# spaceandtimefdn/blitzar

Hardware: NVIDIA H100
Metric: MSM throughput (scalar*point terms/sec), ristretto255, n=2^20 per GPU (higher is better)
Workload: dtype u32 limbs (integer modular arithmetic)

## Files before the change

### blitzar_b200/csrc/msm.cuh

```cuda
#pragma once
#include <algorithm>
#include <vector>

#include "batch_affine.cuh"
#include "curve.cuh"
#include "engine_api.cuh"
#include "lanefield.cuh"

namespace b200 {

struct ColumnDesc {
  const unsigned char* base;
  u64 row_stride;
  u32 bit_offset;
  u32 bit_width;
  u32 n;
  u32 is_signed;
  u32 first_window;
  u32 num_windows;
  u32 table_n;
  u32 gen_base;
};
B200_HD u32 bucket_windows(const ColumnDesc& col) { return col.table_n ? (col.num_windows ? 1u : 0u) : col.num_windows; }

B200_HD void load_scalar_bits(u32 v[8], bool& negative, const ColumnDesc& col, u64 i) {
  const unsigned char* row = col.base + i * col.row_stride;
#pragma unroll
  for (int k = 0; k < 8; ++k)
    v[k] = 0;
  const u32 width = col.bit_width;
  const unsigned char* p = row + (col.bit_offset >> 3);
  const u32 sh = col.bit_offset & 7u;
  if (sh == 0 && width == 256 && (((size_t)p) & 15u) == 0) {
    const uint4* q = (const uint4*)p;
    uint4 a = q[0], b = q[1];
    v[0] = a.x; v[1] = a.y; v[2] = a.z; v[3] = a.w;
    v[4] = b.x; v[5] = b.y; v[6] = b.z; v[7] = b.w;
  } else if (sh == 0 && (width & 31u) == 0 && (((size_t)p) & 3u) == 0) {
    const u32* q = (const u32*)p;
#pragma unroll
    for (int k = 0; k < 8; ++k)
      if ((u32)k < (width >> 5))
        v[k] = q[k];
  } else {
    const u32 nbytes = (sh + width + 7u) >> 3;
#pragma unroll
    for (int k = 0; k < 8; ++k) {
      u64 acc = 0;
#pragma unroll
      for (int b = 0; b < 5; ++b) {
        u32 idx = 4u * k + b;
        if (idx < nbytes)
          acc |= (u64)p[idx] << (8 * b);
      }
      v[k] = (u32)(acc >> sh);
    }
#pragma unroll
    for (int k = 0; k < 8; ++k) {
      int lo = 32 * k;
      if ((int)width <= lo)
        v[k] = 0;
      else if ((int)width < lo + 32)
        v[k] &= (1u << (width - lo)) - 1u;
    }
  }
  negative = false;
  if (col.is_signed) {
    u32 top = width - 1;
    bool neg = false;
#pragma unroll
    for (int k = 0; k < 8; ++k)
      if ((top >> 5) == (u32)k)
        neg = (v[k] >> (top & 31u)) & 1u;
    if (neg) {
      u64 c = 1;
#pragma unroll
      for (int k = 0; k < 8; ++k) {
        int lo = 32 * k;
        u32 m = 0;
        if ((int)width >= lo + 32)
          m = 0xffffffffu;
        else if ((int)width > lo)
          m = (1u << (width - lo)) - 1u;
        c += (u64)((~v[k]) & m);
        v[k] = (u32)c & m;
        c = (m == 0xffffffffu) ? (c >> 32) : 0;
      }
      negative = true;
    }
  }
}

constexpr u32 kAllWindows = 0xffffffffu;
template <class Fn>
B200_HD void for_each_digit(const u32 v[8], bool negative, const ColumnDesc& col, u32 c,
                            u32 nbuckets, Fn f, u32 only_window = kAllWindows) {
  const u32 half = nbuckets;
  const u32 mask = (1u << c) - 1u;
  u64 buf = 0;
  u32 nb = 0, w = 0, carry = 0;
  const u32 W = only_window == kAllWindows
                    ? col.num_windows
                    : (only_window < col.num_windows ? only_window + 1 : 0u);
#pragma unroll
  for (int k = 0; k < 8; ++k) {
    buf |= (u64)v[k] << nb;
    nb += 32;
    while (nb >= c && w < W) {
      u32 d = ((u32)buf & mask) + carry;
      buf >>= c;
      nb -= c;
      bool dneg = d > half;
      carry = dneg ? 1u : 0u;
      if (dneg)
        d = (1u << c) - d;
      if (d && (only_window == kAllWindows || w == only_window))
        f((col.first_window + (col.table_n ? 0u : w)) * nbuckets + (d - 1u), negative != dneg, w);
      ++w;
    }
  }
  while (w < W) {
    u32 d = ((u32)buf & mask) + carry;
    buf >>= c;
    bool dneg = d > half;
    carry = dneg ? 1u : 0u;
    if (dneg)
      d = (1u << c) - d;
    if (d && (only_window == kAllWindows || w == only_window))
      f((col.first_window + (col.table_n ? 0u : w)) * nbuckets + (d - 1u), negative != dneg, w);
    ++w;
  }
}

B200_HD u32 column_of(const u64* col_start, u32 ncols, u64 tid) {
  u32 lo = 0, hi = ncols;
  while (hi - lo > 1) {
    const u32 mid = (lo + hi) >> 1;
    if (tid >= col_start[mid])
      lo = mid;
    else
      hi = mid;
  }
  return lo;
}
struct CountBody {
  static constexpr int kBlock = 256;
  const ColumnDesc* cols;
  const u64* col_start;
  u32 ncols, c, nbuckets;
  u32* counts;
  B200_HD void operator()(u64 tid) const {
    const u32 j = column_of(col_start, ncols, tid);
    const ColumnDesc col = cols[j];
    u64 i = tid - col_start[j];
    u32 v[8];
    bool neg;
    load_scalar_bits(v, neg, col, i);
    u32* cnt = counts;
    for_each_digit(v, neg, col, c, nbuckets, [cnt](u32 key, bool, u32) { B200_ATOMIC_ADD(&cnt[key], 1u); });
  }
};

struct ScatterBody {
  static constexpr int kBlock = 256;
  const ColumnDesc* cols;
  const u64* col_start;
  u32 ncols, c, nbuckets;
  u32* cursor;
  u64* entries;
  u64 total_terms;
  B200_HD void operator()(u64 tid) const {
    u32 only = kAllWindows;
    if (total_terms) {
      only = (u32)(tid / total_terms);
      tid -= (u64)only * total_terms;
    }
    const u32 j = column_of(col_start, ncols, tid);
    const ColumnDesc col = cols[j];
    if (only != kAllWindows && only >= col.num_windows)
      return;
    u64 i = tid - col_start[j];
    u32 v[8];
    bool neg;
    load_scalar_bits(v, neg, col, i);
    u32* cur = cursor;
    u64* en = entries;
    const u32 ii = (u32)i + col.gen_base, tn = col.table_n;
    for_each_digit(v, neg, col, c, nbuckets, [cur, en, ii, tn](u32 key, bool negate, u32 w) {
      u32 pos = B200_ATOMIC_ADD(&cur[key], 1u);
      en[pos] = ((u64)key << 32) | (u64)(((ii + w * tn) << 1) | (negate ? 1u : 0u));
    }, only);
  }
};

constexpr u32 kScanChunk = 256, kScanChunkFirst = 64;
struct ScanUpBody {
  static constexpr int kBlock = 128;
  const u32* in;
  u64 n;
  u32* partial;
  u32 chunk;
  B200_HD void operator()(u64 t) const {
    u64 b = t * chunk, e = b + chunk < n ? b + chunk : n;
    u32 s = 0;
    for (u64 i = b; i < e; ++i)
      s += in[i];
    partial[t] = s;
  }
};
struct ScanTopBody {
  static constexpr int kBlock = 32;
  u32* data;
  u64 n;
  B200_HD void operator()(u64) const {
    u32 s = 0;
    for (u64 i = 0; i < n; ++i) {
      u32 v = data[i];
      data[i] = s;
      s += v;
    }
  }
};
struct ScanDownBody {
  static constexpr int kBlock = 128;
  u32* data;
  u64 n;
  const u32* partial_scanned;
  u32 chunk;
  B200_HD void operator()(u64 t) const {
    u64 b = t * chunk, e = b + chunk < n ? b + chunk : n;
    u32 s = partial_scanned[t];
    for (u64 i = b; i < e; ++i) {
      u32 v = data[i];
      data[i] = s;
      s += v;
    }
  }
};

inline void exclusive_scan(u32* data, u64 n, stream_t s, u32 chunk = kScanChunkFirst) {
  if (n <= kScanChunk) {
    launch(ScanTopBody{data, n}, 1, s);
    return;
  }
  u64 m = (n + chunk - 1) / chunk;
  u32* partial = (u32*)dev_alloc(m * sizeof(u32), s);
  launch(ScanUpBody{data, n, partial, chunk}, m, s);
  exclusive_scan(partial, m, s, kScanChunk);
  launch(ScanDownBody{data, n, partial, chunk}, m, s);
  dev_free(partial, s);
}

#if defined(__CUDACC__) && !defined(B200_EMULATE)
#define B200_BINNED_SORT 1
constexpr u32 kMicroBins = 16384, kBinCap = 8192, kBinSpan = 4096, kMaxBinShift = 12;
constexpr u64 kBinnedSortMinEntries = 1ull << 20;

template <int kBlock> __device__ u32 block_exclusive_scan(u32 v, u32* warp_sums, u32* total) {
  const u32 lane = threadIdx.x & 31u, warp = threadIdx.x >> 5;
  u32 x = v;
#pragma unroll
  for (int d = 1; d < 32; d <<= 1) {
    const u32 y = __shfl_up_sync(0xffffffffu, x, d);
    if (lane >= (u32)d)
      x += y;
  }
  if (lane == 31)
    warp_sums[warp] = x;
  __syncthreads();
  if (warp == 0) {
    u32 w = lane < kBlock / 32 ? warp_sums[lane] : 0u;
#pragma unroll
    for (int d = 1; d < 32; d <<= 1) {
      const u32 y = __shfl_up_sync(0xffffffffu, w, d);
      if (lane >= (u32)d)
        w += y;
    }
    if (lane < kBlock / 32)
      warp_sums[lane] = w;
  }
  __syncthreads();
  const u32 pre = (warp ? warp_sums[warp - 1] : 0u) + x - v;
  *total = warp_sums[kBlock / 32 - 1];
  __syncthreads();
  return pre;
}

template <class Fn>
__device__ void for_each_entry(const ColumnDesc* cols, const u64* col_start, u32 ncols, u32 c,
                               u32 nbuckets, u64 tid, Fn f) {
  const u32 j = column_of(col_start, ncols, tid);
  const ColumnDesc col = cols[j];
  const u64 i = tid - col_start[j];
  u32 v[8];
  bool neg;
  load_scalar_bits(v, neg, col, i);
  const u32 ii = (u32)i + col.gen_base, tn = col.table_n;
  for_each_digit(v, neg, col, c, nbuckets, [&](u32 key, bool negate, u32 w) {
    f(key, ((u64)key << 32) | (u64)(((ii + w * tn) << 1) | (negate ? 1u : 0u)));
  });
}

struct MicroCountBody {
  static constexpr int kBlock = 512;
  const ColumnDesc* cols;
  const u64* col_start;
  u32 ncols, c, nbuckets;
  u64 total_terms;
  u32 tile, shift, nmicro;
  u32* micro_counts;
  __device__ void run(u32 b, unsigned char* smem) const {
    u32* h = (u32*)smem;
    for (u32 m = threadIdx.x; m < nmicro; m += kBlock)
      h[m] = 0;
    __syncthreads();
    const u64 lo = (u64)b * tile, hi = lo + tile < total_terms ? lo + tile : total_terms;
    const u32 sh = shift;
    for (u64 t = lo + threadIdx.x; t < hi; t += kBlock)
      for_each_entry(cols, col_start, ncols, c, nbuckets, t,
                     [h, sh](u32 key, u64) { atomicAdd(&h[key >> sh], 1u); });
    __syncthreads();
    for (u32 m = threadIdx.x; m < nmicro; m += kBlock)
      if (h[m])
        atomicAdd(&micro_counts[m], h[m]);
  }
};

struct PlanBinsBody {
  static constexpr int kBlock = 1024;
  const u32* micro_counts;
  u32 nmicro, span_micro;
  u64 nkeys;
  u32* bin_of;
  u32* bin_start;
  u32* bin_micro;
  u32* bin_cursor;
  u32* nbins_out;
  u32* counts;
  u32* d_m;
  __device__ bool starts_bin(const u32* st, u32 m) const {
    constexpr u32 H = kBinCap / 2;
    return m == 0 || m % span_micro == 0 || micro_counts[m] > H || micro_counts[m - 1] > H ||
           st[m] / H != st[m - 1] / H;
  }
  __device__ void run(u32, unsigned char* smem) const {
    __shared__ u32 ws[32];
    u32* st = (u32*)smem;
    const u32 per = (nmicro + kBlock - 1) / kBlock, m0 = min(threadIdx.x * per, nmicro),
              m1 = min(m0 + per, nmicro);
    u32 sum = 0;
    for (u32 m = m0; m < m1; ++m)
      sum += micro_counts[m];
    u32 total;
    u32 run = block_exclusive_scan<kBlock>(sum, ws, &total);
    for (u32 m = m0; m < m1; ++m) {
      st[m] = run;
      run += micro_counts[m];
    }
    __syncthreads();
    u32 nf = 0;
    for (u32 m = m0; m < m1; ++m)
      nf += starts_bin(st, m) ? 1u : 0u;
    u32 nbins;
    u32 id = block_exclusive_scan<kBlock>(nf, ws, &nbins);
    for (u32 m = m0; m < m1; ++m) {
      if (starts_bin(st, m)) {
        bin_start[id] = st[m];
        bin_micro[id] = m;
        bin_cursor[id] = st[m];
        ++id;
      }
      bin_of[m] = id - 1;
    }
    if (threadIdx.x == 0) {
      bin_start[nbins] = total;
      bin_micro[nbins] = nmicro;
      *nbins_out = nbins;
      counts[nkeys] = total;
      d_m[0] = total;
    }
  }
};

struct CoarseScatterBody {
  static constexpr int kBlock = 1024;
  const ColumnDesc* cols;
  const u64* col_start;
  u32 ncols, c, nbuckets;
  u64 total_terms;
  u32 tile, shift, nmicro;
  const u32* bin_of;
  const u32* nbins_ptr;
  u32* bin_cursor;
  u64* tmp;
  __device__ void run(u32 b, unsigned char* smem) const {
    __shared__ u32 ws[32];
    u32* h = (u32*)smem;
    u32* delta = h + nmicro;
    u64* stage = (u64*)(delta + nmicro + (nmicro & 1u));
    const u32 nbins = *nbins_ptr;
    for (u32 k = threadIdx.x; k < nbins; k += kBlock)
      h[k] = 0;
    __syncthreads();
    const u64 lo = (u64)b * tile, hi = lo + tile < total_terms ? lo + tile : total_terms;
    const u32 sh = shift;
    const u32* map = bin_of;
    for (u64 t = lo + threadIdx.x; t < hi; t += kBlock)
      for_each_entry(cols, col_start, ncols, c, nbuckets, t,
                     [h, sh, map](u32 key, u64) { atomicAdd(&h[__ldg(&map[key >> sh])], 1u); });
    __syncthreads();
    const u32 per = (nbins + kBlock - 1) / kBlock, k0 = min(threadIdx.x * per, nbins),
              k1 = min(k0 + per, nbins);
    u32 sum = 0;
    for (u32 k = k0; k < k1; ++k)
      sum += h[k];
    u32 size;
    u32 run = block_exclusive_scan<kBlock>(sum, ws, &size);
    for (u32 k = k0; k < k1; ++k) {
      const u32 n = h[k];
      if (n)
        delta[k] = atomicAdd(&bin_cursor[k], n) - run;
      h[k] = run;
      run += n;
    }
    __syncthreads();
    for (u64 t = lo + threadIdx.x; t < hi; t += kBlock)
      for_each_entry(cols, col_start, ncols, c, nbuckets, t, [h, sh, map, stage](u32 key, u64 e) {
        stage[atomicAdd(&h[__ldg(&map[key >> sh])], 1u)] = e;
      });
    __syncthreads();
    for (u32 i = threadIdx.x; i < size; i += kBlock) {
      const u64 e = stage[i];
      tmp[delta[__ldg(&map[(u32)(e >> 32) >> sh])] + i] = e;
    }
  }
};

struct BinSortBody {
  static constexpr int kBlock = 1024;
  static constexpr size_t kSmem = 2 * kBinCap * sizeof(u64) + kBinSpan * sizeof(u32);
  const u64* tmp;
  const u32* bin_start;
  const u32* bin_micro;
  const u32* nbins_ptr;
  u32 shift;
  u64 nkeys;
  u64* entries;
  u32* counts;
  __device__ void run(u32 b, unsigned char* smem) const {
    __shared__ u32 ws[32];
    if (b >= *nbins_ptr)
      return;
    u64* ent = (u64*)smem;
    u32* h = (u32*)(smem + 2 * kBinCap * sizeof(u64));
    const u32 lo = bin_start[b], size = bin_start[b + 1] - lo;
    const u64 klo = (u64)bin_micro[b] << shift, khi_m = (u64)bin_micro[b + 1] << shift;
    const u32 span = (u32)((khi_m < nkeys ? khi_m : nkeys) - klo);
    const bool local = size <= kBinCap;
    for (u32 k = threadIdx.x; k < span; k += kBlock)
      h[k] = 0;
    if (local) {
#pragma unroll 4
      for (u32 i = threadIdx.x; i < size; i += kBlock)
        ent[i] = tmp[(u64)lo + i];
    }
    __syncthreads();
    for (u32 i = threadIdx.x; i < size; i += kBlock) {
      const u64 e = local ? ent[i] : tmp[(u64)lo + i];
      atomicAdd(&h[(u32)(e >> 32) - (u32)klo], 1u);
    }
    __syncthreads();
    const u32 per = (span + kBlock - 1) / kBlock, k0 = min(threadIdx.x * per, span),
              k1 = min(k0 + per, span);
    u32 sum = 0;
    for (u32 k = k0; k < k1; ++k)
      sum += h[k];
    u32 total;
    u32 run = block_exclusive_scan<kBlock>(sum, ws, &total);
    for (u32 k = k0; k < k1; ++k) {
      const u32 n = h[k];
      h[k] = run;
      run += n;
      counts[klo + k] = lo + run;
    }
    __syncthreads();
    if (!local) {
      for (u32 i = threadIdx.x; i < size; i += kBlock) {
        const u64 e = tmp[(u64)lo + i];
        entries[(u64)lo + atomicAdd(&h[(u32)(e >> 32) - (u32)klo], 1u)] = e;
      }
      return;
    }
    u64* sorted = ent + kBinCap;
    for (u32 i = threadIdx.x; i < size; i += kBlock) {
      const u64 e = ent[i];
      sorted[atomicAdd(&h[(u32)(e >> 32) - (u32)klo], 1u)] = e;
    }
    __syncthreads();
    for (u32 i = threadIdx.x; i < size; i += kBlock)
      entries[(u64)lo + i] = sorted[i];
  }
};

inline u32 binned_sort_shift(u64 nkeys) {
  u32 shift = 0;
  while ((nkeys + (1ull << shift) - 1) >> shift > kMicroBins)
    ++shift;
  return shift;
}

inline void binned_sort(stream_t s, const ColumnDesc* d_cols, const u64* d_col_start, u32 ncols,
                        u32 c, u32 nbuckets, u64 total_terms, u64 max_entries, u32 max_windows,
                        u64 nkeys, u64* entries, u32* counts, u32* d_m) {
  const u32 shift = binned_sort_shift(nkeys);
  const u32 nmicro = (u32)((nkeys + (1ull << shift) - 1) >> shift);
  const u32 span_micro = std::max(1u, kBinSpan >> shift);
  u32* ws = (u32*)dev_alloc((5ull * nmicro + 3) * sizeof(u32), s);
  u32 *micro_counts = ws, *bin_of = ws + nmicro, *bin_cursor = ws + 2ull * nmicro,
      *bin_start = ws + 3ull * nmicro, *bin_micro = ws + 4ull * nmicro + 1,
      *nbins = ws + 5ull * nmicro + 2;
  u64* tmp = (u64*)dev_alloc(std::max<u64>(max_entries, 1) * sizeof(u64), s);
  dev_zero(micro_counts, nmicro * sizeof(u32), s);
  const u64 count_tile = 4096;
  launch_blocks(MicroCountBody{d_cols, d_col_start, ncols, c, nbuckets, total_terms,
                               (u32)count_tile, shift, nmicro, micro_counts},
                (total_terms + count_tile - 1) / count_tile, nmicro * sizeof(u32), s);
  launch_blocks(PlanBinsBody{micro_counts, nmicro, span_micro, nkeys, bin_of, bin_start, bin_micro,
                             bin_cursor, nbins, counts, d_m},
                1, nmicro * sizeof(u32), s);
  const size_t scatter_smem = 220 * 1024;
  const size_t bin_bytes = (2ull * nmicro + 2) * sizeof(u32);
  const u64 stage_entries = (scatter_smem - bin_bytes) / sizeof(u64);
  const u64 scatter_tile = std::max<u64>(1, stage_entries / max_windows);
  launch_blocks(CoarseScatterBody{d_cols, d_col_start, ncols, c, nbuckets, total_terms,
                                  (u32)scatter_tile, shift, nmicro, bin_of, nbins, bin_cursor, tmp},
                (total_terms + scatter_tile - 1) / scatter_tile, scatter_smem, s);
  launch_blocks(BinSortBody{tmp, bin_start, bin_micro, nbins, shift, nkeys, entries, counts}, nmicro,
                BinSortBody::kSmem, s);
  dev_free(tmp, s);
  dev_free(ws, s);
}
#endif

template <class C> struct FillIdentityBody {
  static constexpr int kBlock = 256;
  static constexpr u32 kChunks = sizeof(typename C::Point) / 16;
  static_assert(sizeof(typename C::Point) % 16 == 0, "points are made of 16-byte aligned fields");
  uint4* p;
  B200_HD void operator()(u64 t) const {
    const typename C::Point id = C::identity();
    const u32 k = (u32)(t % kChunks);
    uint4 v = ((const uint4*)&id)[0];
#pragma unroll
    for (u32 j = 1; j < kChunks; ++j)
      if (j == k)
        v = ((const uint4*)&id)[j];
    p[t] = v;
  }
};
template <class C> inline void fill_identity(stream_t s, typename C::Point* p, u64 n) {
  launch(FillIdentityBody<C>{(uint4*)p}, n * FillIdentityBody<C>::kChunks, s);
}

template <class C> struct MergeBucketsBody {
  static constexpr int kBlock = 128;
  const u32* bucket_end;
  const u32* bucket_begin;
  const typename C::Point* scratch;
  typename C::Point* buckets;
  B200_HD void operator()(u64 k) const {
    const u32 lo = bucket_begin ? bucket_begin[k] : (k ? bucket_end[k - 1] : 0u);
    if (bucket_end[k] == lo)
      return;
    typename C::Point b = buckets[k];
    C::add(b, b, scratch[k]);
    buckets[k] = b;
  }
};

template <class C, bool kGather, class X = SeqExec, bool kUniform = false, bool kUnitZ = false>
struct AccumulateBody {
  static constexpr int kBlock = 128;
  static constexpr int kMinBlocks = !kGather ? 1 : (C::F::N > 8 ? 2 : 3);
  typedef typename C::Point Point;
  typedef typename C::Gen Gen;
  const u32* keys;
  const u64* entries;
  const Gen* gens;
  const Point* pieces;
  const u32* m_ptr;
  u32 K;
  u32 final_level;
  Point* buckets;
  u32* out_keys;
  Point* out_pieces;
  u32* out_m_ptr;
  const u32* unit_veto;

  B200_HD void put_bucket(u32 key, const Point& acc, bool writer) const {
    if (writer)
      buckets[key] = acc;
  }
  B200_HD u32 key_at(u64 i) const { return kGather ? (u32)(entries[i] >> 32) : keys[i]; }
  B200_HD void fetch(Point& acc, u64 i, bool first) const {
    if (kGather) {
      u32 e = (u32)entries[i];
      if (first)
        C::gen_to_point(acc, gens[e >> 1], e & 1u);
      else
        C::template add_gen<X>(acc, acc, gens[e >> 1], e & 1u);
    } else {
      if (first)
        acc = pieces[i];
      else
        C::template add<X>(acc, acc, pieces[i]);
    }
  }
  template <bool kUnit> B200_HD Gen load_gen(u32 idx) const {
    if constexpr (kUnit)
      return C::load_unit_gen(gens + idx);
    else
      return gens[idx];
  }
  template <bool kUnit>
  B200_HD void gather_walk(u64 t, u64 b, u64 e, bool writer, u32& cur, Point& acc,
                           bool& first_seg) const {
    u64 ent = entries[b];
    Gen g = load_gen<kUnit>((u32)ent >> 1);
    cur = (u32)(ent >> 32);
    struct {
      Point p;
      B200_HD void start(const Gen& g, bool negate) { C::gen_to_point(p, g, negate); }
      B200_HD void add(const Gen& g, bool negate) {
        C::template add_gen<X>(p, p, g, negate, kUnit);
      }
      B200_HD void get(Point& out) const { out = p; }
    } ga;
    for (u64 i = b; i < e; ++i) {
      u64 ent_n = ent;
      Gen g_n = g;
      if (i + 1 < e) {
        ent_n = entries[i + 1];
        g_n = load_gen<kUnit>((u32)ent_n >> 1);
      }
      const u32 k = (u32)(ent >> 32);
      const bool negate = ((u32)ent & 1u) != 0;
      if (kUniform) {
        if (i == b) {
          ga.p = C::identity();
        } else if (k != cur) {
          ga.get(acc);
          if (final_level || !first_seg) {
            put_bucket(cur, acc, writer);
          } else if (writer) {
            out_keys[2 * t] = cur;
            out_pieces[2 * t] = acc;
          }
          first_seg = false;
          cur = k;
          ga.p = C::identity();
        }
        ga.add(g, negate);
      } else if (i == b) {
        ga.start(g, negate);
      } else if (k == cur) {
        ga.add(g, negate);
      } else {
        ga.get(acc);
        if (final_level || !first_seg) {
          put_bucket(cur, acc, writer);
        } else if (writer) {
          out_keys[2 * t] = cur;
          out_pieces[2 * t] = acc;
        }
        first_seg = false;
        cur = k;
        ga.start(g, negate);
      }
      ent = ent_n;
      g = g_n;
    }
    ga.get(acc);
  }
  B200_HD void operator()(u64 tid) const {
    const u64 t = tid / X::kLanes;
    const bool writer = (tid % X::kLanes) == 0;
    const u64 M = *m_ptr;
    const u64 T = (M + K - 1) / K;
    if (tid == 0 && out_m_ptr)
      *out_m_ptr = final_level ? 0u : (u32)(2 * T);
    u64 b = t * K;
    if (b >= M)
      return;
    u64 e = b + K < M ? b + K : M;
    u32 cur;
    Point acc;
    bool first_seg = true;
    if (kGather) {
      if (kUnitZ && unit_veto && *unit_veto)
        gather_walk<false>(t, b, e, writer, cur, acc, first_seg);
      else
        gather_walk<kUnitZ>(t, b, e, writer, cur, acc, first_seg);
    } else {
      cur = key_at(b);
      fetch(acc, b, true);
      for (u64 i = b + 1; i < e; ++i) {
        u32 k = key_at(i);
        if (k == cur) {
          fetch(acc, i, false);
        } else {
          if (final_level || !first_seg) {
            put_bucket(cur, acc, writer);
          } else if (writer) {
            out_keys[2 * t] = cur;
            out_pieces[2 * t] = acc;
          }
          first_seg = false;
          cur = k;
          fetch(acc, i, true);
        }
      }
    }
    if (final_level) {
      put_bucket(cur, acc, writer);
      return;
    }
    if (!writer)
      return;
    if (first_seg) {
      out_keys[2 * t] = cur;
      out_pieces[2 * t] = acc;
      out_keys[2 * t + 1] = cur;
      out_pieces[2 * t + 1] = C::identity();
    } else {
      out_keys[2 * t + 1] = cur;
      out_pieces[2 * t + 1] = acc;
    }
  }
};

struct WindowUsedBody {
  static constexpr int kBlock = 64;
  const u32* bucket_end;
  u32 nbuckets;
  u32* window_used;
  B200_HD void operator()(u64 w) const {
    u32 lo = w ? bucket_end[w * nbuckets - 1] : 0u;
    u32 hi = bucket_end[(w + 1) * nbuckets - 1];
    if (hi != lo)
      window_used[w] = 1u;
  }
};

struct WindowUsedFromCountsBody {
  static constexpr int kBlock = 128;
  const u32* counts;
  u64 nkeys;
  u32 nbuckets;
  u32* window_used;
  B200_HD void operator()(u64 t) const {
    const u64 b = t * 256, e = b + 256 < nkeys ? b + 256 : nkeys;
    for (u64 k = b; k < e; ++k)
      if (counts[k])
        window_used[k / nbuckets] = 1u;
  }
};

template <class C, class Ex = SeqExec> struct ReduceBody {
  static constexpr int kBlock = 64;
  typedef typename C::Point Point;
  const Point* X;
  const Point* Cin;
  u32 m_in, g, log2g;
  Point* Xout;
  Point* Cout;
  const u32* window_used;
  u32 nbuckets;
  B200_HD void operator()(u64 tid) const {
    const u64 t = tid / Ex::kLanes;
    const bool writer = (tid % Ex::kLanes) == 0;
    const u32 m_out = m_in / g;
    const u32 w = (u32)(t / m_out), k = (u32)(t % m_out);
    if (window_used[w] == 0) {
      if (writer) {
        Xout[t] = C::identity();
        Cout[t] = C::identity();
      }
      return;
    }
    const Point* x = X + (u64)w * m_in + (u64)k * g;
    Point run = x[g - 1];
    Point acc = Cin ? C::identity() : run;
    if (Cin) {
      acc = run;
      if (g == 1)
        acc = C::identity();
    }
    for (u32 r = g - 1; r-- > 0;) {
      C::template add<Ex>(run, run, x[r]);
      if (r > 0 || !Cin)
        C::template add<Ex>(acc, acc, run);
    }
    if (Cin) {
      const Point* cin = Cin + (u64)w * m_in + (u64)k * g;
      for (u32 r = 0; r < g; ++r)
        C::template add<Ex>(acc, acc, cin[r]);
    }
    for (u32 i = 0; i < log2g; ++i)
      C::template dbl<Ex>(run, run);
    if (writer) {
      Xout[t] = run;
      Cout[t] = acc;
    }
  }
};

template <class C, class X = SeqExec> struct CombineBody {
  static constexpr int kBlock = 32;
  typedef typename C::Point Point;
  const Point* S;
  const ColumnDesc* cols;
  u32 c;
  Point* out;
  B200_HD void operator()(u64 tid) const {
    const u64 j = tid / X::kLanes;
    const bool writer = (tid % X::kLanes) == 0;
    const ColumnDesc col = cols[j];
    if (col.num_windows == 0 || col.n == 0) {
      if (writer)
        out[j] = C::identity();
      return;
    }
    const u32 nw = bucket_windows(col);
    Point acc = S[col.first_window + nw - 1];
    for (u32 w = nw - 1; w-- > 0;) {
      for (u32 i = 0; i < c; ++i)
        C::template dbl<X>(acc, acc);
      C::template add<X>(acc, acc, S[col.first_window + w]);
    }
    if (writer)
      out[j] = acc;
// ... 223 lines not shown
    for (u32 k = kBatchGroup; k-- > 0;) {
      const u64 i = j + k * T;
      if (i >= n)
        continue;
      u64 src, dst;
      map.at(i, src, dst);
      Ed25519::Point p;
      Ed25519::load_point_abi(p, raw + src * Ed25519::kAbiGenBytes);
      if (scale) {
        F::E zi;
        F::mul(zi, inv, pre[i]);
        F::mul(inv, inv, p.Z);
        F::mul(p.X, p.X, zi);
        F::mul(p.Y, p.Y, zi);
        F::mul(p.T, p.T, zi);
        p.Z = F::one();
      }
      Ed25519::Gen g;
      Ed25519::point_to_gen(g, p);
      gens[dst] = g;
    }
  }
};
#ifdef B200_BINNED_SORT
__device__ __forceinline__ F25519::E shfl_up_fe(const F25519::E& a, u32 d) {
  F25519::E r;
#pragma unroll
  for (int k = 0; k < 8; ++k)
    r.l[k] = __shfl_up_sync(0xffffffffu, a.l[k], d);
  return r;
}
__device__ __forceinline__ F25519::E shfl_down_fe(const F25519::E& a, u32 d) {
  F25519::E r;
#pragma unroll
  for (int k = 0; k < 8; ++k)
    r.l[k] = __shfl_down_sync(0xffffffffu, a.l[k], d);
  return r;
}
template <int kBlock>
__device__ void block_prefix_suffix(const F25519::E& x, F25519::E& P, F25519::E& S,
                                    F25519::E& total, F25519::E* ws) {
  typedef F25519 F;
  const u32 lane = threadIdx.x & 31u, warp = threadIdx.x >> 5;
  F::E inc = x, sinc = x;
#pragma unroll
  for (u32 d = 1; d < 32; d <<= 1) {
    const F::E y = shfl_up_fe(inc, d), z = shfl_down_fe(sinc, d);
    if (lane >= d)
      F::mul(inc, inc, y);
    if (lane + d < 32)
      F::mul(sinc, sinc, z);
  }
  F::E pe = shfl_up_fe(inc, 1), se = shfl_down_fe(sinc, 1);
  if (lane == 0)
    pe = F::one();
  if (lane == 31) {
    se = F::one();
    ws[warp] = inc;
  }
  __syncthreads();
  F::E before = F::one(), after = F::one();
  for (u32 w = 0; w < kBlock / 32; ++w) {
    if (w < warp)
      F::mul(before, before, ws[w]);
    else if (w > warp)
      F::mul(after, after, ws[w]);
  }
  F::mul(P, before, pe);
  F::mul(S, se, after);
  F::mul(total, before, ws[warp]);
  F::mul(total, total, after);
  __syncthreads();
}
struct NormalizeUpBlockBody {
  static constexpr int kBlock = kNormBlock;
  typedef F25519 F;
  NormalizeUpBody up;
  F::E* ps;
  F::E* prod;
  __device__ void run(u32 b, unsigned char*) const {
    __shared__ F::E ws[kBlock / 32];
    const u64 j = (u64)b * kBlock + threadIdx.x;
    const F::E g = j < up.T ? up.group(j) : F::one();
    F::E P, S, total;
    block_prefix_suffix<kBlock>(g, P, S, total, ws);
    if (j < up.T)
      F::mul(ps[j], P, S);
    if (threadIdx.x == 0)
      prod[b] = total;
  }
};
struct NormalizeMidBody {
  static constexpr int kBlock = 1024;
  typedef F25519 F;
  F::E* vals;
  F::E* pre;
  u64 m;
  __device__ void run(u32, unsigned char*) const {
    __shared__ F::E ws[kBlock / 32];
    __shared__ F::E inv_total;
    const u64 per = (m + kBlock - 1) / kBlock, lo = min((u64)threadIdx.x * per, m),
              hi = min(lo + per, m);
    F::E c = F::one();
    for (u64 k = lo; k < hi; ++k) {
      pre[k] = c;
      F::mul(c, c, vals[k]);
    }
    F::E P, S, total;
    block_prefix_suffix<kBlock>(c, P, S, total, ws);
    if (threadIdx.x == 0)
      F::invert(inv_total, total);
    __syncthreads();
    F::E inv;
    F::mul(inv, inv_total, P);
    F::mul(inv, inv, S);
    for (u64 k = hi; k-- > lo;) {
      const F::E v = vals[k];
      F::mul(vals[k], inv, pre[k]);
      F::mul(inv, inv, v);
    }
  }
};
#endif
inline void ingest_normalized(stream_t s, const unsigned char* raw, Ed25519::Gen* gens,
                              const IngestMap& map, u64 n, u32* invalid) {
  typedef F25519::E fe;
  if (n == 0)
    return;
  const u64 T = (n + kBatchGroup - 1) / kBatchGroup;
  fe* pre = (fe*)dev_alloc(n * sizeof(fe), s);
  const NormalizeUpBody up{raw, map, n, T, pre, nullptr, invalid};
#ifdef B200_BINNED_SORT
  const u64 blocks = (T + kNormBlock - 1) / kNormBlock;
  fe* ps = (fe*)dev_alloc((T + 2 * blocks) * sizeof(fe), s);
  fe* prod = ps + T;
  launch_blocks(NormalizeUpBlockBody{up, ps, prod}, blocks, 0, s);
  launch_blocks(NormalizeMidBody{prod, prod + blocks, blocks}, 1, 0, s);
  launch(NormalizeDownBody{raw, map, n, T, pre, prod, ps, invalid, gens}, T, s);
  dev_free(ps, s);
#else
  fe* prod = (fe*)dev_alloc(T * sizeof(fe), s);
  NormalizeUpBody u = up;
  u.prod = prod;
  launch(u, T, s);
  batch_invert<F25519>(s, prod, T);
  launch(NormalizeDownBody{raw, map, n, T, pre, prod, nullptr, invalid, gens}, T, s);
  dev_free(prod, s);
#endif
  dev_free(pre, s);
}
template <class C, bool kCommit> struct StoreBody {
  static constexpr int kBlock = 32;
  const typename C::Point* pts;
  unsigned char* out;
  B200_HD void operator()(u64 i) const {
    if (kCommit)
      C::store_commit_abi(out + i * C::kAbiCommitBytes, pts[i]);
    else
      C::store_proj_abi(out + i * C::kAbiProjBytes, pts[i]);
  }
};
template <class C>
inline void launch_store_commit(stream_t s, const typename C::Point* pts, unsigned char* out,
                                u64 count, bool lane_tail) {
#ifdef B200_LANE_TAIL
  if constexpr (C::kCurveId == kRistretto255) {
    if (lane_tail && count && count <= 4096) {
      launch(StoreLaneBody{pts, out, count}, (count + 2) / 3 * 32, s);
      return;
    }
  }
#endif
  launch(StoreBody<C, true>{pts, out}, count, s);
}
template <class C> struct GenToProjBody {
  static constexpr int kBlock = 64;
  const typename C::Gen* gens;
  unsigned char* out;
  B200_HD void operator()(u64 i) const {
    typename C::Point p;
    C::gen_to_point(p, gens[i], false);
    C::store_proj_abi(out + i * C::kAbiProjBytes, p);
  }
};
template <class C> struct SumPartsBody {
  static constexpr int kBlock = 32;
  const typename C::Point* parts;
  u32 nparts, count;
  typename C::Point* out;
  B200_HD void operator()(u64 j) const {
    typename C::Point acc = parts[j];
    for (u32 r = 1; r < nparts; ++r)
      C::add(acc, acc, parts[(u64)r * count + j]);
    out[j] = acc;
  }
};

inline u32 choose_window_bits(u64 max_n, u32 max_width, u32 ncols, size_t point_bytes) {
  const double kMaxBucketBytes = 3.0e9;
  u32 best = 2;
  double best_cost = 1e300;
  for (u32 c = 2; c <= 16; ++c) {
    double W = (double)(max_width / c + 1);
    if (c > 8 && W * (double)(1u << (c - 1)) * (double)ncols * (double)point_bytes > kMaxBucketBytes)
      break;
    double cost = W * ((double)max_n + 2.5 * (double)(1u << (c - 1)));
    if (cost < best_cost) {
      best_cost = cost;
      best = c;
    }
  }
  return best;
}

struct MsmPlan {
  u32 c = 0, nbuckets = 0, ncols = 0, total_windows = 0;
  u64 nkeys = 0, max_n = 0, total_terms = 0, total_entries = 0;
  std::vector<ColumnDesc> cols;
};

inline MsmPlan msm_make_plan(std::vector<ColumnDesc> cols, const MsmOptions& opt,
                             size_t point_bytes) {
  MsmPlan p;
  p.ncols = (u32)cols.size();
  u32 max_width = 1;
  for (auto& col : cols) {
    p.max_n = std::max<u64>(p.max_n, col.n);
    p.total_terms += col.n;
    if (col.n)
      max_width = std::max(max_width, col.bit_width);
  }
  p.c = opt.window_bits ? opt.window_bits
                        : choose_window_bits(p.max_n, max_width, p.ncols, point_bytes);
  p.nbuckets = 1u << (p.c - 1);
  u64 max_entries = 0;
  for (auto& col : cols) {
    col.first_window = p.total_windows;
    col.num_windows = col.n ? col.bit_width / p.c + 1 : 0;
    p.total_windows += bucket_windows(col);
    max_entries += (u64)col.n * col.num_windows;
    if (col.table_n)
      B200_REQUIRE((u64)col.table_n * col.num_windows < (1ull << 31), "generator table too large");
    if (col.n)
      B200_REQUIRE((u64)col.gen_base + col.n + (u64)(col.num_windows - 1) * col.table_n < (1ull << 31),
                   "generator index of a column too large");
  }
  p.nkeys = (u64)p.total_windows * p.nbuckets;
  p.total_entries = max_entries;
  B200_REQUIRE(p.nkeys < (1ull << 32), "too many buckets for one pass");
  p.cols = std::move(cols);
  return p;
}

struct StagedRange {
  const ColumnDesc* d_cols = nullptr;
  const u64* d_col_start = nullptr;
  u64 total_terms = 0, max_entries = 0;
  u32 max_windows = 0;
  StagedRange(stream_t s, const MsmPlan& plan, u64 begin, u64 end) {
    const u32 ncols = plan.ncols;
    std::vector<ColumnDesc> cols(plan.cols);
    std::vector<u64> col_start(ncols + 1, 0);
    for (u32 j = 0; j < ncols; ++j) {
      u64 lo = std::min<u64>(begin, cols[j].n), hi = std::min<u64>(end, cols[j].n);
      cols[j].base += lo * cols[j].row_stride;
      cols[j].n = (u32)(hi - lo);
      col_start[j + 1] = col_start[j] + cols[j].n;
      max_entries += (u64)cols[j].n * cols[j].num_windows;
      max_windows = std::max(max_windows, cols[j].n ? cols[j].num_windows : 0u);
    }
    total_terms = col_start[ncols];
    if (total_terms == 0)
      return;
    B200_REQUIRE(max_entries < (1ull << 32) && end - begin < (1ull << 31),
                 "too many (term, window) entries for one sort pass");
    const size_t desc_bytes = ncols * sizeof(ColumnDesc), start_bytes = (ncols + 1) * sizeof(u64);
    std::vector<unsigned char> stage(desc_bytes + start_bytes);
    std::memcpy(stage.data(), cols.data(), desc_bytes);
    std::memcpy(stage.data() + desc_bytes, col_start.data(), start_bytes);
    d_cols = (const ColumnDesc*)stage_to_device(s, stage.data(), stage.size());
    d_col_start = (const u64*)((const unsigned char*)d_cols + desc_bytes);
  }
};

struct SortedLayout {
  u64* entries;
  u32* counts;
  u32* starts;
  u32* d_m;
  u64 slots_max;
  bool binned;
};

inline SortedLayout sort_entries(stream_t s, const MsmPlan& plan, const StagedRange& r, u32 L,
                                 const MsmOptions& opt, u32* window_used) {
  const u32 ncols = plan.ncols, c = plan.c, nbuckets = plan.nbuckets;
  const u64 nkeys = plan.nkeys, max_entries = r.max_entries, total_terms = r.total_terms;
  SortedLayout out{};
  out.slots_max = L ? ((max_entries + nkeys * ((1ull << L) - 1) + (1ull << L) - 1) >> L) << L : max_entries;
  out.counts = (u32*)dev_alloc((nkeys + 1) * sizeof(u32), s);
  out.d_m = (u32*)dev_alloc(16 * sizeof(u32), s);
  out.entries = (u64*)dev_alloc(out.slots_max * sizeof(u64), s);
#ifdef B200_BINNED_SORT
  out.binned = L == 0 && opt.sort_path != 0 && binned_sort_shift(nkeys) <= kMaxBinShift &&
               (opt.sort_path == 2 || max_entries >= kBinnedSortMinEntries);
  if (out.binned)
    binned_sort(s, r.d_cols, r.d_col_start, ncols, c, nbuckets, total_terms, max_entries,
                r.max_windows, nkeys, out.entries, out.counts, out.d_m);
#endif
  if (!out.binned) {
    dev_zero(out.counts, (nkeys + 1) * sizeof(u32), s);
    launch(CountBody{r.d_cols, r.d_col_start, ncols, c, nbuckets, out.counts}, total_terms, s);
    if (L) {
      launch(WindowUsedFromCountsBody{out.counts, nkeys, nbuckets, window_used}, (nkeys + 255) / 256, s);
      launch(PadCountsBody{out.counts, (1u << L) - 1u}, nkeys, s);
    }
    exclusive_scan(out.counts, nkeys + 1, s);
    copy_d2d(out.d_m, out.counts + nkeys, sizeof(u32), s);
    if (L) {
      out.starts = (u32*)dev_alloc((nkeys + 1) * sizeof(u32), s);
      copy_d2d(out.starts, out.counts, (nkeys + 1) * sizeof(u32), s);
    }
    const bool window_major = opt.scatter_window_major && r.max_windows > 1;
    launch(ScatterBody{r.d_cols, r.d_col_start, ncols, c, nbuckets, out.counts, out.entries,
                       window_major ? total_terms : 0},
           window_major ? total_terms * r.max_windows : total_terms, s);
  }
  if (L)
    launch(FillPadsBody{out.starts, out.counts, out.entries}, nkeys, s);
  else
    launch(WindowUsedBody{out.counts, nbuckets, window_used}, plan.total_windows, s);
  return out;
}

inline unsigned sort_selftest(stream_t s, std::vector<ColumnDesc> cols, u32 c) {
  MsmOptions opt;
  opt.window_bits = c;
  const MsmPlan plan = msm_make_plan(std::move(cols), opt, 160);
  const StagedRange r(s, plan, 0, plan.max_n);
  if (r.total_terms == 0)
    return ~0u;
  const u64 nkeys = plan.nkeys, M = r.max_entries;
  DevBuf<u32> window_used(plan.total_windows, s);
  opt.sort_path = 0;
  const SortedLayout a = sort_entries(s, plan, r, 0, opt, window_used.p);
  opt.sort_path = 2;
  const SortedLayout b = sort_entries(s, plan, r, 0, opt, window_used.p);
  std::vector<u32> ca(nkeys + 1), cb(nkeys + 1), m(1);
  std::vector<u64> ea(M), eb(M);
  copy_d2h(ca.data(), a.counts, (nkeys + 1) * sizeof(u32), s);
  copy_d2h(cb.data(), b.counts, (nkeys + 1) * sizeof(u32), s);
  copy_d2h(m.data(), b.d_m, sizeof(u32), s);
  copy_d2h(ea.data(), a.entries, M * sizeof(u64), s);
  copy_d2h(eb.data(), b.entries, M * sizeof(u64), s);
  stream_sync(s);
  for (void* p : {(void*)a.entries, (void*)a.counts, (void*)a.d_m, (void*)b.entries, (void*)b.counts,
                  (void*)b.d_m, (void*)r.d_cols})
    dev_free(p, s);
  if (!b.binned)
    return ~0u;
  unsigned bad = m[0] == ca[nkeys] ? 0u : 1u;
  for (u64 k = 0; k < nkeys; ++k) {
    const u32 lo = k ? ca[k - 1] : 0u, hi = ca[k];
    if (cb[k] != hi || hi < lo || hi > M) {
      ++bad;
      continue;
    }
    std::sort(ea.begin() + lo, ea.begin() + hi);
    std::sort(eb.begin() + lo, eb.begin() + hi);
    if (!std::equal(ea.begin() + lo, ea.begin() + hi, eb.begin() + lo))
      ++bad;
  }
  return bad;
}

struct RangeHook {
  virtual void before_range(u64 begin, u64 end) = 0;
  virtual void before_accumulate() {}
  virtual ~RangeHook() {}
};

template <class C>
stream_t chunk_walk(stream_t s, stream_t tail, WalkInput<C> walk, u32* d_m, bool unit,
                    const u32* unit_veto, typename C::Point* target, const MsmOptions& opt,
                    std::vector<void*>& to_free) {
  typedef typename C::Point Point;
  u32 K = opt.chunk1 ? std::max(opt.chunk1, 4u) : (walk.m_max >= (1ull << 23) ? 64u : 32u);
  const u32 chunkn = std::max(opt.chunkn, 4u);
  const u32* lvl_keys = nullptr;
  const Point* lvl_pieces = nullptr;
  stream_t cs = s;
  for (int level = 0;; ++level) {
    const bool final_level = walk.m_max <= K;
    u64 T = (walk.m_max + K - 1) / K;
    u32* out_keys = final_level ? nullptr : (u32*)dev_alloc(2 * T * sizeof(u32), cs);
    Point* out_pieces = final_level ? nullptr : (Point*)dev_alloc(2 * T * sizeof(Point), cs);
    to_free.insert(to_free.end(), {out_keys, out_pieces});
    u32* out_m = d_m + 1 + (level % 8);
    if (level == 0) {
      const bool uniform =
          opt.uniform_add == 2 ? C::kCurveId == kRistretto255 : opt.uniform_add != 0;
      constexpr bool kEd = C::kCurveId == kRistretto255;
      const bool unit_path = kEd && unit;
      if (uniform && unit_path)
        launch(AccumulateBody<C, true, SeqExec, true, kEd>{nullptr, walk.entries, walk.gens, nullptr,
                                                            walk.m_ptr, K, final_level, target,
                                                            out_keys, out_pieces, out_m, unit_veto},
               T, s);
      else if (uniform)
        launch(AccumulateBody<C, true, SeqExec, true>{nullptr, walk.entries, walk.gens, nullptr,
                                                      walk.m_ptr, K, final_level, target, out_keys,
                                                      out_pieces, out_m, nullptr},
               T, s);
      else if (unit_path)
        launch(AccumulateBody<C, true, SeqExec, false, kEd>{nullptr, walk.entries, walk.gens, nullptr,
                                                             walk.m_ptr, K, final_level, target,
                                                             out_keys, out_pieces, out_m, unit_veto},
               T, s);
      else
        launch(AccumulateBody<C, true>{nullptr, walk.entries, walk.gens, nullptr, walk.m_ptr, K,
                                       final_level, target, out_keys, out_pieces, out_m, nullptr},
               T, s);
      KernelTimer::get().end(s);
      if (tail != s)
        stream_follow(tail, s);
      cs = tail;
    } else if (T <= opt.quad_threshold) {
      launch(AccumulateBody<C, false, QuadExec>{lvl_keys, nullptr, nullptr, lvl_pieces, walk.m_ptr,
                                                K, final_level, target, out_keys, out_pieces, out_m,
                                                nullptr},
             T * QuadExec::kLanes, cs);
    } else {
      launch(AccumulateBody<C, false>{lvl_keys, nullptr, nullptr, lvl_pieces, walk.m_ptr, K,
                                      final_level, target, out_keys, out_pieces, out_m, nullptr},
             T, cs);
    }
    if (final_level)
      break;
    lvl_keys = out_keys;
    lvl_pieces = out_pieces;
    walk.m_ptr = out_m;
    walk.m_max = 2 * T;
    K = chunkn;
  }
  return cs;
}

template <class C>
void msm_accumulate_range(stream_t s, const MsmPlan& plan, const typename C::Gen* gens, u64 begin,
                          u64 end, bool add_into, typename C::Point* d_buckets,
                          u32* d_window_used, const MsmOptions& opt, stream_t tail,
                          RangeHook* hook = nullptr) {
  const StagedRange r(s, plan, begin, end);
  if (r.total_terms == 0)
    return;
  gens += begin;
  StageRange nvtx_sort("msm: digit count + scan + scatter");
  const u64 max_entries = r.max_entries, nkeys = plan.nkeys;
  u32 L = 0;
  if constexpr (C::kBatchAffine) {
    const double mean = (double)max_entries / (double)nkeys;
    if (opt.pair_levels >= 0)
      L = (u32)opt.pair_levels;
    else if (max_entries >= (1ull << 23))
      while (L < 6 && (double)(32u << L) <= mean)
        ++L;
    while (L > 0 && max_entries + nkeys * ((1ull << L) - 1) >= (1ull << 32) - (1ull << L))
      --L;
  }
  const SortedLayout sorted = sort_entries(s, plan, r, L, opt, d_window_used);
  B200_LOG(3, "range [%llu, %llu): %llu terms, %llu entries max, c=%u, %llu keys, pair levels %u",
           (unsigned long long)begin, (unsigned long long)end, (unsigned long long)r.total_terms,
           (unsigned long long)max_entries, plan.c, (unsigned long long)nkeys, L);
  WalkInput<C> walk{gens, sorted.entries, sorted.d_m, max_entries};
  std::vector<void*> to_free;
  if (hook)
    hook->before_accumulate();
  KernelTimer::get().begin(s);
  StageRange nvtx_acc("msm: bucket accumulation");
  if constexpr (C::kBatchAffine) {
    if (L) {
      walk = run_pair_levels<C>(s, L, sorted.entries, gens, sorted.d_m, sorted.slots_max,
                                opt.pair_batch);
      to_free = {(void*)walk.gens, (void*)walk.entries};
    }
  }
  typedef typename C::Point Point;
  Point* target = add_into ? (Point*)dev_alloc(nkeys * sizeof(Point), s) : d_buckets;
  const bool unit = walk.gens == gens && opt.gens_normalized;
  const stream_t cs =
      chunk_walk<C>(s, tail, walk, sorted.d_m, unit, opt.unit_veto, target, opt, to_free);
  if (add_into) {
    launch(MergeBucketsBody<C>{sorted.counts, sorted.starts, target, d_buckets}, nkeys, cs);
    dev_free(target, cs);
  }
  to_free.insert(to_free.end(), {sorted.d_m, sorted.counts, sorted.starts});
  for (void* ptr : to_free)
    dev_free(ptr, cs);
  dev_free(sorted.entries, s);
  dev_free((void*)r.d_cols, s);
}

template <class C>
void msm_finish(stream_t s, const MsmPlan& plan, const typename C::Point* d_buckets,
                const u32* d_window_used, typename C::Point* out, const MsmOptions& opt) {
  typedef typename C::Point Point;
  StageRange nvtx_fin("msm: bucket reduction + window combination");
  const u32 total_windows = plan.total_windows, nbuckets = plan.nbuckets, ncols = plan.ncols;
  ColumnDesc* d_cols =
      (ColumnDesc*)stage_to_device(s, plan.cols.data(), ncols * sizeof(ColumnDesc));
  Point* d_S = nullptr;
  u32 m = nbuckets;
  const Point* X = d_buckets;
  const Point* Cin = nullptr;
  std::vector<void*> to_free;
  if (m == 1) {
    d_S = (Point*)dev_alloc(total_windows * sizeof(Point), s);
    copy_d2d(d_S, d_buckets, total_windows * sizeof(Point), s);
  }
  bool first = true;
  while (m > 1) {
    u32 g = first ? std::min<u32>(opt.reduce_g1, m) : std::min<u32>(opt.reduce_gn, m);
    u32 log2g = 0;
    while ((1u << log2g) < g)
      ++log2g;
    u32 m_out = m / g;
    Point* Xout = (Point*)dev_alloc((u64)total_windows * m_out * sizeof(Point), s);
    Point* Cout = (Point*)dev_alloc((u64)total_windows * m_out * sizeof(Point), s);
    if ((u64)total_windows * m_out <= opt.quad_threshold)
      launch(ReduceBody<C, QuadExecConv>{X, Cin, m, g, log2g, Xout, Cout, d_window_used, nbuckets},
             (u64)total_windows * m_out * QuadExec::kLanes, s);
    else
      launch(ReduceBody<C>{X, Cin, m, g, log2g, Xout, Cout, d_window_used, nbuckets},
             (u64)total_windows * m_out, s);
    to_free.push_back(Xout);
    if (m_out > 1)
      to_free.push_back(Cout);
    X = Xout;
    Cin = Cout;
    m = m_out;
    first = false;
    if (m == 1)
      d_S = Cout;
  }
  for (void* ptr : to_free)
    dev_free(ptr, s);
  bool uniform_windows = true;
  for (u32 j = 1; j < ncols; ++j)
    uniform_windows = uniform_windows && bucket_windows(plan.cols[j]) == bucket_windows(plan.cols[0]);
#ifdef B200_LANE_TAIL
  bool lane_done = false;
  if constexpr (C::kCurveId == kRistretto255) {
    if (ncols <= 2048 && opt.lane_tail) {
      launch(CombineLaneBody{d_S, d_cols, plan.c, out}, (u64)ncols * 32, s);
      lane_done = true;
    }
  }
  if (lane_done) {
  } else
#endif
  if (ncols <= opt.quad_threshold && uniform_windows)
    launch(CombineBody<C, QuadExecConv>{d_S, d_cols, plan.c, out}, (u64)ncols * QuadExec::kLanes,
           s);
  else if (ncols <= opt.quad_threshold)
    launch(CombineBody<C, QuadExec>{d_S, d_cols, plan.c, out}, (u64)ncols * QuadExec::kLanes, s);
  else
    launch(CombineBody<C>{d_S, d_cols, plan.c, out}, ncols, s);
  dev_free(d_S, s);
  dev_free(d_cols, s);
}

template <class C>
void msm_run(stream_t s, const typename C::Gen* gens, std::vector<ColumnDesc> cols,
             typename C::Point* out, const MsmOptions& opt = MsmOptions(), u32 num_ranges = 1,
             RangeHook* hook = nullptr, stream_t tail = stream_t()) {
  typedef typename C::Point Point;
  if (cols.empty())
    return;
  MsmPlan plan = msm_make_plan(std::move(cols), opt, sizeof(Point));
  B200_LOG(2, "msm: curve %u, %u columns, longest %llu, %llu terms, window %u bits, %u bucket sets%s",
           C::kCurveId, plan.ncols, (unsigned long long)plan.max_n,
           (unsigned long long)plan.total_terms, plan.c, plan.total_windows,
           plan.ncols && plan.cols[0].table_n ? " (fixed-base table)" : "");
  if (plan.total_terms == 0 || plan.total_windows == 0) {
    if (hook)
      hook->before_range(0, plan.max_n);
    fill_identity<C>(s, out, plan.ncols);
    return;
  }
  Point* d_buckets = (Point*)dev_alloc(plan.nkeys * sizeof(Point), s);
  fill_identity<C>(s, d_buckets, plan.nkeys);
  u32* d_window_used = (u32*)dev_alloc(plan.total_windows * sizeof(u32), s);
  dev_zero(d_window_used, plan.total_windows * sizeof(u32), s);
  if (num_ranges < 1)
    num_ranges = 1;
  const u64 limit = opt.max_range_entries ? opt.max_range_entries : (1ull << 31);
  const u64 needed = (plan.total_entries + limit - 1) / limit;
  if (needed > num_ranges)
    num_ranges = (u32)std::min<u64>(needed, plan.max_n);
  const bool overlap = num_ranges > 1 && tail != stream_t() && tail != s;
  for (u32 r = 0; r < num_ranges; ++r) {
    u64 begin = range_begin(plan.max_n, r, num_ranges, opt.range_skew),
        end = range_begin(plan.max_n, r + 1, num_ranges, opt.range_skew);
    if (hook)
      hook->before_range(begin, end);
    msm_accumulate_range<C>(s, plan, gens, begin, end, r > 0, d_buckets, d_window_used, opt,
                            overlap ? tail : s, hook);
  }
  if (overlap)
    stream_follow(s, tail);
  msm_finish<C>(s, plan, d_buckets, d_window_used, out, opt);
// ... 6 lines not shown
```

Measured before the change: 337.8 million.

## Stage entries once in coarse scatter and sort by 16-bit index permutation

The coarse scatter kernel now stages each decoded entry once into shared memory at a fixed (term, window) slot, instead of decoding the scalar digits twice. It then builds a 16-bit order permutation for the bin-grouped write-out. The bin sort likewise replaces its second 64-bit sorted buffer with a 16-bit order array, which halves its shared memory so two blocks can fit per SM. A plan function bounds the number of bins, caches the micro-to-bin map in shared memory as 16-bit values, and sizes tiles and grids to that bound. The cost is an extra shared-memory pass with indirect reads and sentinel initialisation, plus tighter 16-bit indexing limits.

```diff
diff --git a/blitzar_b200/csrc/msm.cuh b/blitzar_b200/csrc/msm.cuh
--- a/blitzar_b200/csrc/msm.cuh
+++ b/blitzar_b200/csrc/msm.cuh
@@ -254,6 +254,7 @@
 #if defined(__CUDACC__) && !defined(B200_EMULATE)
 #define B200_BINNED_SORT 1
 constexpr u32 kMicroBins = 16384, kBinCap = 8192, kBinSpan = 4096, kMaxBinShift = 12;
+constexpr size_t kBlockSmemMax = 227 * 1024;
 constexpr u64 kBinnedSortMinEntries = 1ull << 20;
 
 template <int kBlock> __device__ u32 block_exclusive_scan(u32 v, u32* warp_sums, u32* total) {
@@ -297,7 +298,7 @@
   load_scalar_bits(v, neg, col, i);
   const u32 ii = (u32)i + col.gen_base, tn = col.table_n;
   for_each_digit(v, neg, col, c, nbuckets, [&](u32 key, bool negate, u32 w) {
-    f(key, ((u64)key << 32) | (u64)(((ii + w * tn) << 1) | (negate ? 1u : 0u)));
+    f(key, ((u64)key << 32) | (u64)(((ii + w * tn) << 1) | (negate ? 1u : 0u)), w);
   });
 }
 
@@ -318,7 +319,7 @@
     const u32 sh = shift;
     for (u64 t = lo + threadIdx.x; t < hi; t += kBlock)
       for_each_entry(cols, col_start, ncols, c, nbuckets, t,
-                     [h, sh](u32 key, u64) { atomicAdd(&h[key >> sh], 1u); });
+                     [h, sh](u32 key, u64, u32) { atomicAdd(&h[key >> sh], 1u); });
     __syncthreads();
     for (u32 m = threadIdx.x; m < nmicro; m += kBlock)
       if (h[m])
@@ -384,30 +385,46 @@
 
 struct CoarseScatterBody {
   static constexpr int kBlock = 1024;
+  static constexpr u64 kNoEntry = ~0ull;
+  static constexpr size_t kSlotBytes = sizeof(u64) + sizeof(unsigned short), kBinBytes = 2 * sizeof(u32),
+                          kMicroBytes = sizeof(unsigned short);
+  static_assert(kMicroBins <= 65536, "bins are indexed by 16 bits");
+  static constexpr size_t kSmem = kBlockSmemMax - 32 * sizeof(u32);
+  static_assert(kSmem / kSlotBytes <= 65536, "stage slots are indexed by 16 bits");
   const ColumnDesc* cols;
   const u64* col_start;
   u32 ncols, c, nbuckets;
   u64 total_terms;
-  u32 tile, shift, nmicro;
+  u32 tile, windows, shift, max_bins, nmicro;
   const u32* bin_of;
   const u32* nbins_ptr;
   u32* bin_cursor;
   u64* tmp;
   __device__ void run(u32 b, unsigned char* smem) const {
     __shared__ u32 ws[32];
-    u32* h = (u32*)smem;
-    u32* delta = h + nmicro;
-    u64* stage = (u64*)(delta + nmicro + (nmicro & 1u));
+    const u32 slots = tile * windows;
+    u64* stage = (u64*)smem;
+    u32* h = (u32*)(stage + slots);
+    u32* delta = h + max_bins;
+    unsigned short* order = (unsigned short*)(delta + max_bins);
+    unsigned short* map = order + slots;
     const u32 nbins = *nbins_ptr;
     for (u32 k = threadIdx.x; k < nbins; k += kBlock)
       h[k] = 0;
+    for (u32 m = threadIdx.x; m < nmicro; m += kBlock)
+      map[m] = (unsigned short)bin_of[m];
+    for (u32 i = threadIdx.x; i < slots; i += kBlock)
+      stage[i] = kNoEntry;
     __syncthreads();
     const u64 lo = (u64)b * tile, hi = lo + tile < total_terms ? lo + tile : total_terms;
-    const u32 sh = shift;
-    const u32* map = bin_of;
-    for (u64 t = lo + threadIdx.x; t < hi; t += kBlock)
-      for_each_entry(cols, col_start, ncols, c, nbuckets, t,
-                     [h, sh, map](u32 key, u64) { atomicAdd(&h[__ldg(&map[key >> sh])], 1u); });
+    const u32 sh = shift, tl = tile;
+    for (u64 t = lo + threadIdx.x; t < hi; t += kBlock) {
+      const u32 s0 = (u32)(t - lo);
+      for_each_entry(cols, col_start, ncols, c, nbuckets, t, [=](u32 key, u64 e, u32 w) {
+        stage[s0 + w * tl] = e;
+        atomicAdd(&h[map[key >> sh]], 1u);
+      });
+    }
     __syncthreads();
     const u32 per = (nbins + kBlock - 1) / kBlock, k0 = min(threadIdx.x * per, nbins),
               k1 = min(k0 + per, nbins);
@@ -424,21 +441,23 @@
       run += n;
     }
     __syncthreads();
-    for (u64 t = lo + threadIdx.x; t < hi; t += kBlock)
-      for_each_entry(cols, col_start, ncols, c, nbuckets, t, [h, sh, map, stage](u32 key, u64 e) {
-        stage[atomicAdd(&h[__ldg(&map[key >> sh])], 1u)] = e;
-      });
+    for (u32 i = threadIdx.x; i < slots; i += kBlock) {
+      const u64 e = stage[i];
+      if (e != kNoEntry)
+        order[atomicAdd(&h[map[(u32)(e >> 32) >> sh]], 1u)] = (unsigned short)i;
+    }
     __syncthreads();
     for (u32 i = threadIdx.x; i < size; i += kBlock) {
-      const u64 e = stage[i];
-      tmp[delta[__ldg(&map[(u32)(e >> 32) >> sh])] + i] = e;
+      const u64 e = stage[order[i]];
+      tmp[delta[map[(u32)(e >> 32) >> sh]] + i] = e;
     }
   }
 };
 
 struct BinSortBody {
   static constexpr int kBlock = 1024;
-  static constexpr size_t kSmem = 2 * kBinCap * sizeof(u64) + kBinSpan * sizeof(u32);
+  static constexpr size_t kSmem = kBinCap * (sizeof(u64) + sizeof(unsigned short)) + kBinSpan * sizeof(u32);
+  static_assert(kSmem + 32 * sizeof(u32) + 1024 <= 228 * 1024 / 2, "two bin sorts per SM");
   const u64* tmp;
   const u32* bin_start;
   const u32* bin_micro;
@@ -452,7 +471,8 @@
     if (b >= *nbins_ptr)
       return;
     u64* ent = (u64*)smem;
-    u32* h = (u32*)(smem + 2 * kBinCap * sizeof(u64));
+    u32* h = (u32*)(smem + kBinCap * sizeof(u64));
+    unsigned short* order = (unsigned short*)(h + kBinSpan);
     const u32 lo = bin_start[b], size = bin_start[b + 1] - lo;
     const u64 klo = (u64)bin_micro[b] << shift, khi_m = (u64)bin_micro[b + 1] << shift;
     const u32 span = (u32)((khi_m < nkeys ? khi_m : nkeys) - klo);
@@ -491,14 +511,11 @@
       }
       return;
     }
-    u64* sorted = ent + kBinCap;
-    for (u32 i = threadIdx.x; i < size; i += kBlock) {
-      const u64 e = ent[i];
-      sorted[atomicAdd(&h[(u32)(e >> 32) - (u32)klo], 1u)] = e;
-    }
+    for (u32 i = threadIdx.x; i < size; i += kBlock)
+      order[atomicAdd(&h[(u32)(ent[i] >> 32) - (u32)klo], 1u)] = (unsigned short)i;
     __syncthreads();
     for (u32 i = threadIdx.x; i < size; i += kBlock)
-      entries[(u64)lo + i] = sorted[i];
+      entries[(u64)lo + i] = ent[order[i]];
   }
 };
 
@@ -509,12 +526,34 @@
   return shift;
 }
 
-inline void binned_sort(stream_t s, const ColumnDesc* d_cols, const u64* d_col_start, u32 ncols,
-                        u32 c, u32 nbuckets, u64 total_terms, u64 max_entries, u32 max_windows,
-                        u64 nkeys, u64* entries, u32* counts, u32* d_m) {
-  const u32 shift = binned_sort_shift(nkeys);
-  const u32 nmicro = (u32)((nkeys + (1ull << shift) - 1) >> shift);
-  const u32 span_micro = std::max(1u, kBinSpan >> shift);
+struct BinnedSortPlan {
+  u32 shift = 0, nmicro = 0, span_micro = 0;
+  u32 max_bins = 0;
+  u32 tile = 0;
+};
+inline BinnedSortPlan binned_sort_plan(u64 nkeys, u64 max_entries, u32 max_windows) {
+  BinnedSortPlan p;
+  p.shift = binned_sort_shift(nkeys);
+  if (p.shift > kMaxBinShift)
+    return p;
+  p.nmicro = (u32)((nkeys + (1ull << p.shift) - 1) >> p.shift);
+  p.span_micro = std::max(1u, kBinSpan >> p.shift);
+  constexpr u64 H = kBinCap / 2;
+  const u64 cuts = (p.nmicro + p.span_micro - 1) / p.span_micro + max_entries / H + max_entries / (H + 1);
+  p.max_bins = (u32)std::min<u64>(p.nmicro, cuts);
+  using CS = CoarseScatterBody;
+  const size_t bin_bytes = (size_t)p.max_bins * CS::kBinBytes + (size_t)p.nmicro * CS::kMicroBytes;
+  const size_t slots = bin_bytes < CS::kSmem ? (CS::kSmem - bin_bytes) / CS::kSlotBytes : 0;
+  if (slots >= (size_t)CS::kBlock)
+    p.tile = (u32)(slots / std::max(1u, max_windows));
+  return p;
+}
+
+inline void binned_sort(stream_t s, const BinnedSortPlan& p, const ColumnDesc* d_cols,
+                        const u64* d_col_start, u32 ncols, u32 c, u32 nbuckets, u64 total_terms,
+                        u64 max_entries, u32 max_windows, u64 nkeys, u64* entries, u32* counts,
+                        u32* d_m) {
+  const u32 shift = p.shift, nmicro = p.nmicro, span_micro = p.span_micro;
   u32* ws = (u32*)dev_alloc((5ull * nmicro + 3) * sizeof(u32), s);
   u32 *micro_counts = ws, *bin_of = ws + nmicro, *bin_cursor = ws + 2ull * nmicro,
       *bin_start = ws + 3ull * nmicro, *bin_micro = ws + 4ull * nmicro + 1,
@@ -528,15 +567,15 @@
   launch_blocks(PlanBinsBody{micro_counts, nmicro, span_micro, nkeys, bin_of, bin_start, bin_micro,
                              bin_cursor, nbins, counts, d_m},
                 1, nmicro * sizeof(u32), s);
-  const size_t scatter_smem = 220 * 1024;
-  const size_t bin_bytes = (2ull * nmicro + 2) * sizeof(u32);
-  const u64 stage_entries = (scatter_smem - bin_bytes) / sizeof(u64);
-  const u64 scatter_tile = std::max<u64>(1, stage_entries / max_windows);
-  launch_blocks(CoarseScatterBody{d_cols, d_col_start, ncols, c, nbuckets, total_terms,
-                                  (u32)scatter_tile, shift, nmicro, bin_of, nbins, bin_cursor, tmp},
-                (total_terms + scatter_tile - 1) / scatter_tile, scatter_smem, s);
-  launch_blocks(BinSortBody{tmp, bin_start, bin_micro, nbins, shift, nkeys, entries, counts}, nmicro,
-                BinSortBody::kSmem, s);
+  const size_t scatter_smem = (size_t)p.tile * max_windows * CoarseScatterBody::kSlotBytes +
+                              (size_t)p.max_bins * CoarseScatterBody::kBinBytes +
+                              (size_t)nmicro * CoarseScatterBody::kMicroBytes;
+  launch_blocks(CoarseScatterBody{d_cols, d_col_start, ncols, c, nbuckets, total_terms, p.tile,
+                                  max_windows, shift, p.max_bins, nmicro, bin_of, nbins, bin_cursor, tmp},
+                (total_terms + p.tile - 1) / p.tile, scatter_smem, s);
+  const bool dense = max_entries > (u64)nmicro * (kBinCap / 2);
+  launch_blocks(BinSortBody{tmp, bin_start, bin_micro, nbins, shift, nkeys, entries, counts},
+                p.max_bins, dense ? kBlockSmemMax - 32 * sizeof(u32) : BinSortBody::kSmem, s);
   dev_free(tmp, s);
   dev_free(ws, s);
 }
@@ -1366,11 +1405,14 @@
   out.d_m = (u32*)dev_alloc(16 * sizeof(u32), s);
   out.entries = (u64*)dev_alloc(out.slots_max * sizeof(u64), s);
 #ifdef B200_BINNED_SORT
-  out.binned = L == 0 && opt.sort_path != 0 && binned_sort_shift(nkeys) <= kMaxBinShift &&
-               (opt.sort_path == 2 || max_entries >= kBinnedSortMinEntries);
-  if (out.binned)
-    binned_sort(s, r.d_cols, r.d_col_start, ncols, c, nbuckets, total_terms, max_entries,
-                r.max_windows, nkeys, out.entries, out.counts, out.d_m);
+  out.binned = L == 0 && opt.sort_path != 0 && (opt.sort_path == 2 || max_entries >= kBinnedSortMinEntries);
+  if (out.binned) {
+    const BinnedSortPlan bp = binned_sort_plan(nkeys, max_entries, r.max_windows);
+    out.binned = bp.tile != 0;
+    if (out.binned)
+      binned_sort(s, bp, r.d_cols, r.d_col_start, ncols, c, nbuckets, total_terms, max_entries,
+                  r.max_windows, nkeys, out.entries, out.counts, out.d_m);
+  }
 #endif
   if (!out.binned) {
     dev_zero(out.counts, (nkeys + 1) * sizeof(u32), s);
```

Measured after the change: 349.1 million (median of 6 runs). +3.4%, better.
